# vovach777/llcomp

Hardware: AMD Instinct MI355X
Metric: encode+decode MPix/s on 4K RGB8, bit-exact (higher is better)
Workload: dtype int32

## Files before the change

llcomp_amd/csrc/model_kernels.hip:

```cpp
#include <algorithm>

#include "device_common.hpp"
#include "kernels.hpp"

namespace llcomp_mi {

namespace {

constexpr int kMW = 256;
constexpr int kMH = 32;

template <int C>
__device__ __forceinline__ void rct_forward(const uint8_t* p, int16_t (&o)[C]) {
    if constexpr (C >= 3) {
        const int g = p[1], cb = int(p[2]) - g, cr = int(p[0]) - g;
        o[0] = int16_t(cr);
        o[1] = int16_t(g + (cb + cr) / 4);
        o[2] = int16_t(cb);
        if constexpr (C == 4) o[3] = p[3];
    } else {
#pragma unroll
        for (int k = 0; k < C; ++k) o[k] = p[k];
    }
}
// ... 500 lines not shown
constexpr uint32_t kSegPieceDwords = 4096;
__global__ __launch_bounds__(256) void k_copy_segments(const uint8_t* __restrict__ src, uint8_t* __restrict__ dst,
                                                       const uint64_t* __restrict__ src_off, const uint64_t* __restrict__ dst_off,
                                                       const uint64_t* __restrict__ len) {
    const uint64_t n = len[blockIdx.y];
    const uint8_t* s = src + src_off[blockIdx.y];
    uint8_t* d = dst + dst_off[blockIdx.y];
    const uint64_t head = min(n, uint64_t((4 - (reinterpret_cast<uintptr_t>(d) & 3)) & 3));
    const uint64_t ndw = (n - head) >> 2, tail = (n - head) & 3;
    for (uint64_t j0 = uint64_t(blockIdx.x) * kSegPieceDwords; j0 < ndw; j0 += uint64_t(gridDim.x) * kSegPieceDwords) {
        const uint64_t j1 = min(ndw, j0 + kSegPieceDwords);
        for (uint64_t j = j0 + threadIdx.x; j < j1; j += 256) {
            uint32_t w;
            __builtin_memcpy(&w, s + head + 4 * j, 4);
            *reinterpret_cast<uint32_t*>(d + head + 4 * j) = w;
        }
    }
    if (blockIdx.x == 0) {
        if (threadIdx.x < head) d[threadIdx.x] = s[threadIdx.x];
        if (threadIdx.x < tail) d[head + 4 * ndw + threadIdx.x] = s[head + 4 * ndw + threadIdx.x];
    }
}

__global__ __launch_bounds__(256) void k_range_sums(const uint32_t* __restrict__ vals, const uint64_t* __restrict__ start,
                                                    const uint64_t* __restrict__ count, uint64_t* __restrict__ out, uint32_t cap) {
    __shared__ unsigned long long part[4];
    const uint64_t s = start[blockIdx.x], n = count[blockIdx.x];
    unsigned long long acc = 0;
    for (uint64_t j = threadIdx.x; j < n; j += 256) acc += min(vals[s + j], cap);
    for (int o = 32; o > 0; o >>= 1) acc += __shfl_down(acc, o);
    if ((threadIdx.x & 63) == 0) part[threadIdx.x >> 6] = acc;
    __syncthreads();
    if (threadIdx.x == 0) out[blockIdx.x] = part[0] + part[1] + part[2] + part[3];
}

struct SliceSpan {
    unsigned long long origin;
    uint32_t n_row;
    uint32_t n;
};
__device__ __forceinline__ void load_spans(const Geometry& g, uint32_t group, SliceSpan* spans) {
    if (threadIdx.x < 64) {
        const uint32_t id = (group << g.lane_shift) + threadIdx.x;
        SliceSpan sp{0, 1, 0};
        if (threadIdx.x < (1u << g.lane_shift) && id < g.n_slices) {
            const SliceRect r = slice_rect(g, id);
            sp.origin = slice_origin(g, r);
            sp.n_row = r.sw * g.nch;
            sp.n = sp.n_row * r.sh;
        }
        spans[threadIdx.x] = sp;
    }
    __syncthreads();
}
__device__ __forceinline__ size_t span_index(const SliceSpan& sp, uint32_t k, size_t row_stride) {
    const uint32_t y = k / sp.n_row;
    return size_t(sp.origin) + size_t(y) * row_stride + (k - y * sp.n_row);
}

template <typename T>
__global__ __launch_bounds__(256) void k_to_lane_order(const Geometry g, const uint32_t max_n,
                                                       const T* __restrict__ img, T* __restrict__ lanes) {
    __shared__ SliceSpan spans[64];
    __shared__ T tile[64][65];
    const uint32_t chunks = (max_n + 63) / 64;
    const uint32_t group = blockIdx.x / chunks, k0 = (blockIdx.x - group * chunks) * 64;
    load_spans(g, group, spans);
    const size_t rs = slice_row_stride(g);
    const uint32_t a = threadIdx.x & 63, b = threadIdx.x >> 6;
    {
        T v[16];
#pragma unroll
        for (int t = 0; t < 16; ++t) {
            const SliceSpan sp = spans[b + 4 * t];
            const uint32_t k = k0 + a;
            v[t] = k < sp.n ? img[span_index(sp, k, rs)] : T(0);
        }
#pragma unroll
        for (int t = 0; t < 16; ++t) tile[b + 4 * t][a] = v[t];
    }
    __syncthreads();
    const uint32_t gw = 1u << g.lane_shift;
    T* out = lanes + ((size_t(group) * max_n + k0) << g.lane_shift);
    const uint32_t n_el = min(64u, max_n - k0) << g.lane_shift;
    for (uint32_t el = threadIdx.x; el < n_el; el += 256) out[el] = tile[el & (gw - 1)][el >> g.lane_shift];
}

template <typename T>
__global__ __launch_bounds__(256) void k_from_lane_order(const Geometry g, const uint32_t max_n,
                                                         const T* __restrict__ lanes, T* __restrict__ img) {
    __shared__ SliceSpan spans[64];
    __shared__ T tile[64][65];
    const uint32_t chunks = (max_n + 63) / 64;
    const uint32_t group = blockIdx.x / chunks, k0 = (blockIdx.x - group * chunks) * 64;
    load_spans(g, group, spans);
    const size_t rs = slice_row_stride(g);
    const uint32_t a = threadIdx.x & 63, b = threadIdx.x >> 6;
    const uint32_t gw = 1u << g.lane_shift;
    const T* in = lanes + ((size_t(group) * max_n + k0) << g.lane_shift);
    const uint32_t n_el = min(64u, max_n - k0) << g.lane_shift;
    {
        T v[16];
#pragma unroll
        for (int t = 0; t < 16; ++t) {
            const uint32_t el = threadIdx.x + 256 * t;
            v[t] = el < n_el ? in[el] : T(0);
        }
#pragma unroll
        for (int t = 0; t < 16; ++t) {
            const uint32_t el = threadIdx.x + 256 * t;
            if (el < (64u << g.lane_shift)) tile[el & (gw - 1)][el >> g.lane_shift] = v[t];
        }
    }
    __syncthreads();
    for (uint32_t j = b; j < 64; j += 4) {
        const SliceSpan sp = spans[j];
        const uint32_t k = k0 + a;
        if (k < sp.n) img[span_index(sp, k, rs)] = tile[j][a];
    }
}

constexpr uint32_t kXcds = 8;
__device__ __forceinline__ bool xcd_group_chunk(uint32_t n_groups, uint32_t chunks, uint32_t& group, uint32_t& chunk) {
    const uint32_t xcd = blockIdx.x % kXcds, slot = blockIdx.x / kXcds;
    group = (slot / chunks) * kXcds + xcd;
    chunk = slot - (slot / chunks) * chunks;
    return group < n_groups;
}
__host__ inline uint64_t xcd_grid(uint32_t n_groups, uint32_t chunks) { return uint64_t((n_groups + kXcds - 1) / kXcds) * kXcds * chunks; }
__device__ __forceinline__ bool xcd_chunk_group(uint32_t n_groups, uint32_t chunks, uint32_t& group, uint32_t& chunk) {
    const uint32_t xcd = blockIdx.x % kXcds, slot = blockIdx.x / kXcds;
    const uint32_t per_class = (chunks + kXcds - 1) / kXcds;
    group = slot / per_class;
    chunk = xcd + kXcds * (slot - group * per_class);
    return group < n_groups && chunk < chunks;
}
__host__ inline uint64_t xcd_chunk_grid(uint32_t n_groups, uint32_t chunks) { return uint64_t(n_groups) * ((chunks + kXcds - 1) / kXcds) * kXcds; }

template <int C>
__device__ __forceinline__ void rct_pixel(const uint8_t* p, int (&v)[C]) {
    if constexpr (C >= 3) {
        const int g = p[1], cb = int(p[2]) - g, cr = int(p[0]) - g;
        v[0] = cr;
        v[1] = g + (cb + cr) / 4;
        v[2] = cb;
        if constexpr (C == 4) v[3] = p[3];
    } else {
#pragma unroll
        for (int k = 0; k < C; ++k) v[k] = p[k];
    }
}
struct RowTile {
    unsigned long long base;
    uint32_t sw;
};
template <int C>
__device__ __forceinline__ void load_row_tiles(const Geometry& g, uint32_t first_tile, uint32_t ntiles, RowTile* tiles) {
    if (threadIdx.x < ntiles) {
        const uint32_t tile = first_tile + threadIdx.x;
        const uint32_t per_frame = g.ntx * g.nty;
        const uint32_t frame = tile / per_frame, rem = tile - frame * per_frame;
        const uint32_t y = rem / g.ntx, tx = rem - y * g.ntx;
        const uint32_t x0 = tx * g.tile_w;
        tiles[threadIdx.x].base = ((size_t(frame) * g.h + y) * g.w + x0) * C;
        tiles[threadIdx.x].sw = g.w - x0 < g.tile_w ? g.w - x0 : g.tile_w;
    }
}

typedef short s16x2 __attribute__((ext_vector_type(2)));
typedef unsigned short u16x2 __attribute__((ext_vector_type(2)));
__device__ __forceinline__ u16x2 pk_min_u16(u16x2 a, u16x2 b) {
    u16x2 d;
    asm("v_pk_min_u16 %0, %1, %2" : "=v"(d) : "v"(a), "v"(b));
    return d;
}

template <int C>
__global__ __launch_bounds__(256) void k_model_rows_fwd(const Geometry g, const uint8_t* __restrict__ px,
                                                        uint16_t* __restrict__ lanes) {
    constexpr int K = 64, RUN = (K + 2) * C, TPG = 64 / C + 2;
    constexpr int RUNW = (RUN + 3) / 4 + 1;
    constexpr int PADL = (C - 1 + 1) & ~1, OCOLS = (PADL + 64 + C - 1 + 1) & ~1;
    __shared__ uint32_t raw[TPG][RUNW + 1];
    __shared__ __attribute__((aligned(4))) uint16_t otile[K][OCOLS];
    __shared__ RowTile tiles[TPG];
    const uint32_t chunks = (g.tile_w + K - 1) / K;
    uint32_t group, chunk;
    if (!xcd_group_chunk((g.n_slices + (1u << g.lane_shift) - 1) >> g.lane_shift, chunks, group, chunk)) return;
    const uint32_t k0 = chunk * K;
    const uint32_t gw = 1u << g.lane_shift;
    const uint32_t first_id = group << g.lane_shift;
    const uint32_t end_id = first_id + gw < g.n_slices ? first_id + gw : g.n_slices;
    const uint32_t first_tile = first_id / C, ntiles = (end_id - 1) / C - first_tile + 1;
    load_row_tiles<C>(g, first_tile, ntiles, tiles);
    __syncthreads();
    const size_t total_bytes = size_t(g.frames) * g.h * g.w * C;
    const uint32_t lane = threadIdx.x & 63, wave = threadIdx.x >> 6;
    constexpr int TPW = (TPG + 3) / 4, DPT = (RUNW + 63) / 64;
    uint32_t got[TPW][DPT];
#pragma unroll
    for (int t = 0; t < TPW; ++t) {
        const uint32_t tt = wave + 4 * t;
#pragma unroll
        for (int e = 0; e < DPT; ++e) got[t][e] = 0;
        if (tt < ntiles) {
            const long long start = (long long)tiles[tt].base + (long long)(int(k0) - 2) * C;
            const unsigned long long a0u = (unsigned long long)(start & ~3ll);
            const long long a0 = (long long)((unsigned long long)uint32_t(__builtin_amdgcn_readfirstlane(uint32_t(a0u))) |
                                             ((unsigned long long)uint32_t(__builtin_amdgcn_readfirstlane(uint32_t(a0u >> 32))) << 32));
            if (a0 >= 0 && size_t(a0) + 4 * size_t(RUNW) <= total_bytes) {
#pragma unroll
                for (int e = 0; e < DPT; ++e) {
                    const uint32_t d = lane + 64 * e;
                    if (d < uint32_t(RUNW)) __builtin_memcpy(&got[t][e], px + a0 + 4 * d, 4);
                }
            } else {
#pragma unroll
                for (int e = 0; e < DPT; ++e) {
                    const long long al = a0 + 4ll * (lane + 64 * e);
                    if (al >= 0 && size_t(al) + 4 <= total_bytes) __builtin_memcpy(&got[t][e], px + al, 4);
                    else if (al >= 0 && size_t(al) < total_bytes) got[t][e] = load_bytes_le(px + al, uint32_t(total_bytes - size_t(al)));
                }
            }
        }
    }
#pragma unroll
    for (int t = 0; t < TPW; ++t) {
        const uint32_t tt = wave + 4 * t;
#pragma unroll
        for (int e = 0; e < DPT; ++e) {
            const uint32_t d = lane + 64 * e;
            if (tt < ntiles && d < uint32_t(RUNW)) raw[tt][d] = got[t][e];
        }
    }
    __syncthreads();
    const uint32_t q = threadIdx.x & 7;
    const bool small = (g.flags & kGeoSmallModel) != 0;
    for (uint32_t tt = threadIdx.x >> 3; tt < ntiles; tt += 32) {
        const uint32_t sw = tiles[tt].sw;
        const uint32_t kb = k0 + 8 * q;
        if (kb >= sw) continue;
        const uint32_t skew = uint32_t(((long long)tiles[tt].base + (long long)(int(k0) - 2) * C) & 3);
        const uint8_t* p = reinterpret_cast<const uint8_t*>(&raw[tt][0]) + skew + 8 * q * C;
        s16x2 V[C][5];
#pragma unroll
        for (int j = 0; j < 5; ++j) {
            const uint8_t* a = p + 2 * j * C;
            if constexpr (C >= 3) {
                const s16x2 R = {short(a[0]), short(a[C])}, G = {short(a[1]), short(a[C + 1])}, B = {short(a[2]), short(a[C + 2])};
                const s16x2 cr = R - G, cb = B - G, sum = cb + cr;
                V[0][j] = cr;
                V[1][j] = G + ((sum + ((sum >> 15) & short(3))) >> 2);
                V[2][j] = cb;
                if constexpr (C == 4) V[3][j] = s16x2{short(a[3]), short(a[C + 3])};
            } else {
#pragma unroll
                for (int ch = 0; ch < C; ++ch) V[ch][j] = s16x2{short(a[ch]), short(a[C + ch])};
            }
        }
        uint32_t first_mask = ~0u;
        if (kb == 0) {
            first_mask = 0;
#pragma unroll
            for (int ch = 0; ch < C; ++ch) V[ch][0] = s16x2{128, 128};
        }
        if (small) first_mask = 0;
        const uint32_t colp = uint32_t(int((first_tile + tt) * C) - int(first_id) + PADL);
#pragma unroll
        for (int m = 0; m < 4; ++m) {
#pragma unroll
            for (int ch = 0; ch < C; ++ch) {
                const s16x2 cur = V[ch][m + 1], Lp = V[ch][m];
                const s16x2 lp = {V[ch][m].y, V[ch][m + 1].x};
                s16x2 dq = Lp - lp;
                uint32_t dqb = __builtin_bit_cast(uint32_t, dq) & ((m == 0 || small) ? first_mask : ~0u);
                dq = __builtin_bit_cast(s16x2, dqb);
                const s16x2 neg = dq >> 15;
                const u16x2 aq = __builtin_bit_cast(u16x2, (dq ^ neg) - neg);
                const u16x2 one = {1, 1};
                const u16x2 cidx = pk_min_u16(aq, one) + pk_min_u16(aq >> 2, one);
                const s16x2 res = ((cur - lp) ^ neg) - neg;
                const u16x2 sym = (__builtin_bit_cast(u16x2, res) & (unsigned short)0xFFF) + (cidx << 12);
                otile[8 * q + 2 * m][colp + ch] = sym.x;
                otile[8 * q + 2 * m + 1][colp + ch] = sym.y;
            }
        }
    }
    __syncthreads();
    if (g.lane_shift == 6) {
        for (uint32_t i = threadIdx.x; i < uint32_t(K) * 32; i += 256) {
            const uint32_t kk = i >> 5, d = i & 31, k = k0 + kk;
            if (k < g.tile_w)
                *reinterpret_cast<uint32_t*>(lanes + lane_order_index(g, first_id + 2 * d, k)) =
                    *reinterpret_cast<const uint32_t*>(&otile[kk][PADL + 2 * d]);
        }
    } else {
        for (uint32_t i = threadIdx.x; i < uint32_t(K) * gw; i += 256) {
            const uint32_t kk = i / gw, col = i - kk * gw, k = k0 + kk;
            if (k < g.tile_w && first_id + col < end_id) lanes[lane_order_index(g, first_id + col, k)] = otile[kk][PADL + col];
        }
    }
}

template <int C>
__global__ __launch_bounds__(256) void k_model_rows_inv(const Geometry g, const int16_t* __restrict__ lanes,
                                                        uint8_t* __restrict__ px) {
    constexpr int K = 64, TPG = 64 / C + 2;
    __shared__ __attribute__((aligned(4))) int16_t tile[K][64 + C + 1 + ((C + 1) & 1)];
    __shared__ RowTile tiles[TPG];
    const uint32_t chunks = (g.tile_w + K - 1) / K;
    uint32_t group, chunk;
    if (!xcd_chunk_group((g.n_slices + (1u << g.lane_shift) - 1) >> g.lane_shift, chunks, group, chunk)) return;
    const uint32_t k0 = chunk * K;
    const uint32_t gw = 1u << g.lane_shift;
    const uint32_t first_id = group << g.lane_shift;
    const uint32_t end_id = first_id + gw < g.n_slices ? first_id + gw : g.n_slices;
    const uint32_t first_tile = (first_id + C - 1) / C;
    const uint32_t end_tile = (end_id + C - 1) / C;
    if (first_tile >= end_tile) return;
    const uint32_t ntiles = end_tile - first_tile;
    load_row_tiles<C>(g, first_tile, ntiles, tiles);
    {
        uint32_t w[K * 32 / 256];
#pragma unroll
        for (int it = 0; it < K * 32 / 256; ++it) {
            const uint32_t i = threadIdx.x + 256 * it, kk = i >> 5, d = i & 31, k = k0 + kk;
            w[it] = 0;
            if (k < g.tile_w && g.lane_shift == 6)
                w[it] = *reinterpret_cast<const uint32_t*>(lanes + lane_order_index(g, first_id + 2 * d, k));
        }
        static_assert(K * (C - 1) <= 256, "one extra lane sample per thread");
        const uint32_t xk = threadIdx.x / (C > 1 ? C - 1 : 1), xe = threadIdx.x - xk * (C - 1);
        int16_t x = 0;
        if constexpr (C > 1) {
            const uint32_t id = first_id + gw + xe;
            if (xk < uint32_t(K) && id < g.n_slices && k0 + xk < g.tile_w) x = lanes[lane_order_index(g, id, k0 + xk)];
        }
#pragma unroll
        for (int it = 0; it < K * 32 / 256; ++it) {
            const uint32_t i = threadIdx.x + 256 * it, kk = i >> 5, d = i & 31;
            *reinterpret_cast<uint32_t*>(&tile[kk][2 * d]) = w[it];
        }
        if (g.lane_shift != 6) {
            __syncthreads();
            for (uint32_t i = threadIdx.x; i < uint32_t(K) * gw; i += 256) {
                const uint32_t kk = i / gw, col = i - kk * gw, k = k0 + kk;
                tile[kk][col] = (first_id + col < g.n_slices && k < g.tile_w) ? lanes[lane_order_index(g, first_id + col, k)] : int16_t(0);
            }
        }
        if constexpr (C > 1) {
            if (xk < uint32_t(K)) tile[xk][gw + xe] = x;
        }
    }
    __syncthreads();
    const uint32_t col0 = first_tile * C - first_id;
    const uint32_t q4 = threadIdx.x & 15;
    for (uint32_t tt = threadIdx.x >> 4; tt < ntiles; tt += 16) {
        const uint32_t sw = tiles[tt].sw, kb = k0 + 4 * q4;
        if (kb >= sw) continue;
        uint8_t bytes[4 * C];
#pragma unroll
        for (int i = 0; i < 4; ++i) {
            const int16_t* s = &tile[4 * q4 + i][col0 + tt * C];
            if constexpr (C >= 3) {
                int r = s[0], gg = s[1], bb = s[2];
                gg -= (r + bb) / 4;
                r += gg;
                bb += gg;
                bytes[i * C + 0] = uint8_t(min(max(r, 0), 255));
                bytes[i * C + 1] = uint8_t(min(max(gg, 0), 255));
                bytes[i * C + 2] = uint8_t(min(max(bb, 0), 255));
                if constexpr (C == 4) bytes[i * C + 3] = uint8_t(s[3]);
            } else {
#pragma unroll
                for (int c = 0; c < C; ++c) bytes[i * C + c] = uint8_t(s[c]);
            }
        }
        uint8_t* o = px + tiles[tt].base + size_t(kb) * C;
        const uint32_t npx = sw - kb < 4 ? sw - kb : 4;
        if (npx == 4) {
            uint32_t w[C];
#pragma unroll
            for (int c = 0; c < C; ++c)
                w[c] = uint32_t(bytes[4 * c]) | (uint32_t(bytes[4 * c + 1]) << 8) | (uint32_t(bytes[4 * c + 2]) << 16) |
                       (uint32_t(bytes[4 * c + 3]) << 24);
            __builtin_memcpy(o, w, 4 * C);
        } else {
            for (uint32_t i = 0; i < npx * C; ++i) o[i] = bytes[i];
        }
    }
}

struct RowTileCrop {
    long long base;
    uint32_t klo, khi;
};
template <int C>
__device__ __forceinline__ void load_row_tiles_crop(const Geometry& g, uint32_t first_tile, uint32_t ntiles, const Crop& cr,
                                                    RowTileCrop* tiles) {
    if (threadIdx.x < ntiles) {
        const uint32_t tile = first_tile + threadIdx.x;
        const uint32_t per_frame = g.ntx * g.nty;
        const uint32_t frame = tile / per_frame, rem = tile - frame * per_frame;
        const uint32_t y = rem / g.ntx, tx = rem - y * g.ntx;
        const uint32_t x0 = tx * g.tile_w;
        const uint32_t sw = g.w - x0 < g.tile_w ? g.w - x0 : g.tile_w;
        const uint32_t klo = cr.x0 > x0 ? cr.x0 - x0 : 0u;
        uint32_t khi = cr.x0 + cr.rw > x0 ? min(sw, cr.x0 + cr.rw - x0) : 0u;
        if (y < cr.y0 || y >= cr.y0 + cr.rh || khi <= klo) khi = 0;
        tiles[threadIdx.x].base = ((long long)(size_t(frame) * cr.rh + (y - cr.y0)) * cr.rw + (long long)x0 - (long long)cr.x0) * C;
        tiles[threadIdx.x].klo = klo;
        tiles[threadIdx.x].khi = khi;
    }
}
template <int C>
__global__ __launch_bounds__(256) void k_model_rows_inv_crop(const Geometry g, const int16_t* __restrict__ lanes,
                                                             uint8_t* __restrict__ px, const Crop cr) {
    constexpr int K = 64, TPG = 64 / C + 2;
    __shared__ __attribute__((aligned(4))) int16_t tile[K][64 + C + 1 + ((C + 1) & 1)];
    __shared__ RowTileCrop tiles[TPG];
    const uint32_t chunks = (g.tile_w + K - 1) / K;
    uint32_t group, chunk;
    if (!xcd_chunk_group((g.n_slices + (1u << g.lane_shift) - 1) >> g.lane_shift, chunks, group, chunk)) return;
    const uint32_t k0 = chunk * K;
    const uint32_t gw = 1u << g.lane_shift;
    const uint32_t first_id = group << g.lane_shift;
    const uint32_t end_id = first_id + gw < g.n_slices ? first_id + gw : g.n_slices;
    const uint32_t first_tile = (first_id + C - 1) / C;
    const uint32_t end_tile = (end_id + C - 1) / C;
    if (first_tile >= end_tile) return;
    const uint32_t ntiles = end_tile - first_tile;
    load_row_tiles_crop<C>(g, first_tile, ntiles, cr, tiles);
    {
        uint32_t w[K * 32 / 256];
#pragma unroll
        for (int it = 0; it < K * 32 / 256; ++it) {
            const uint32_t i = threadIdx.x + 256 * it, kk = i >> 5, d = i & 31, k = k0 + kk;
            w[it] = 0;
            if (k < g.tile_w && g.lane_shift == 6)
                w[it] = *reinterpret_cast<const uint32_t*>(lanes + lane_order_index(g, first_id + 2 * d, k));
        }
#pragma unroll
        for (int it = 0; it < K * 32 / 256; ++it) {
            const uint32_t i = threadIdx.x + 256 * it, kk = i >> 5, d = i & 31;
            *reinterpret_cast<uint32_t*>(&tile[kk][2 * d]) = w[it];
        }
    }
    if (g.lane_shift != 6) {
        __syncthreads();
        for (uint32_t i = threadIdx.x; i < uint32_t(K) * gw; i += 256) {
            const uint32_t kk = i / gw, col = i - kk * gw, k = k0 + kk;
            tile[kk][col] = (first_id + col < g.n_slices && k < g.tile_w) ? lanes[lane_order_index(g, first_id + col, k)] : int16_t(0);
        }
    }
    if constexpr (C > 1) {
        for (uint32_t i = threadIdx.x; i < uint32_t(K) * (C - 1); i += 256) {
            const uint32_t kk = i / (C - 1), e = i - kk * (C - 1), k = k0 + kk;
            const uint32_t id = first_id + gw + e;
            tile[kk][gw + e] = (id < g.n_slices && k < g.tile_w) ? lanes[lane_order_index(g, id, k)] : int16_t(0);
        }
    }
    __syncthreads();
    const uint32_t col0 = first_tile * C - first_id;
    const uint32_t q4 = threadIdx.x & 15;
    for (uint32_t tt = threadIdx.x >> 4; tt < ntiles; tt += 16) {
        const uint32_t sw = tiles[tt].khi, klo = tiles[tt].klo, kb = k0 + 4 * q4;
        if (kb >= sw || kb + 4 <= klo) continue;
        uint8_t bytes[4 * C];
#pragma unroll
        for (int i = 0; i < 4; ++i) {
            const int16_t* s = &tile[4 * q4 + i][col0 + tt * C];
            if constexpr (C >= 3) {
                int r = s[0], gg = s[1], bb = s[2];
                gg -= (r + bb) / 4;
                r += gg;
                bb += gg;
                bytes[i * C + 0] = uint8_t(min(max(r, 0), 255));
                bytes[i * C + 1] = uint8_t(min(max(gg, 0), 255));
                bytes[i * C + 2] = uint8_t(min(max(bb, 0), 255));
                if constexpr (C == 4) bytes[i * C + 3] = uint8_t(s[3]);
            } else {
#pragma unroll
                for (int c = 0; c < C; ++c) bytes[i * C + c] = uint8_t(s[c]);
            }
        }
        const uint32_t npx = sw - kb < 4 ? sw - kb : 4;
        if (npx < 4 || kb < klo) {
            for (uint32_t i = kb < klo ? klo - kb : 0u; i < npx; ++i)
                for (uint32_t c = 0; c < uint32_t(C); ++c) px[tiles[tt].base + (long long)(kb + i) * C + c] = bytes[i * C + c];
            continue;
        }
        uint32_t w[C];
#pragma unroll
        for (int c = 0; c < C; ++c)
            w[c] = uint32_t(bytes[4 * c]) | (uint32_t(bytes[4 * c + 1]) << 8) | (uint32_t(bytes[4 * c + 2]) << 16) |
                   (uint32_t(bytes[4 * c + 3]) << 24);
        __builtin_memcpy(px + tiles[tt].base + size_t(kb) * C, w, 4 * C);
    }
}



__global__ __launch_bounds__(256) void k_regions_index(const Geometry full, const Geometry sub, const RegionsFrame* __restrict__ tab,
                                                       const uint32_t* __restrict__ slice_len, const uint64_t* __restrict__ group_off,
                                                       uint32_t* __restrict__ sub_len, uint64_t* __restrict__ sub_off) {
    const uint32_t j = blockIdx.x * 256 + threadIdx.x;
    if (j >= sub.n_slices) return;
    const uint32_t id = regions_full_id(full, sub, tab, j);
    unsigned long long o = group_off[id >> full.lane_shift];
    for (uint32_t i = id & ~((1u << full.lane_shift) - 1); i < id; ++i) o += slice_len[i];
    sub_len[j] = slice_len[id];
    sub_off[j] = o;
}

template <int C>
__global__ __launch_bounds__(256) void k_model_inv_crops(const Geometry g, const int16_t* __restrict__ rec, uint8_t* __restrict__ px,
                                                         const RegionsFrame* __restrict__ tab, uint32_t rw, uint32_t rh, size_t npix) {
    const uint32_t c = C ? uint32_t(C) : g.c;
    const size_t per_frame = size_t(rw) * rh;
    for (size_t i = size_t(blockIdx.x) * blockDim.x + threadIdx.x; i < npix; i += size_t(gridDim.x) * blockDim.x) {
        const uint32_t f = uint32_t(i / per_frame);
        const uint32_t rem = uint32_t(i - f * per_frame), yy = rem / rw, xx = rem - yy * rw;
        const uint32_t y = tab[f].cy0 + yy, x = tab[f].cx0 + xx;
        uint8_t* o = px + (size_t(tab[f].out) * per_frame + rem) * c;
        uint32_t k = 0;
        if (c >= 3) {
            int r = rec[sample_index(g, f, y, x, 0)], gg = rec[sample_index(g, f, y, x, 1)], b = rec[sample_index(g, f, y, x, 2)];
            gg -= (r + b) / 4;
            r += gg;
            b += gg;
            o[0] = uint8_t(min(max(r, 0), 255));
            o[1] = uint8_t(min(max(gg, 0), 255));
            o[2] = uint8_t(min(max(b, 0), 255));
            k = 3;
        }
        for (; k < c; ++k) o[k] = uint8_t(rec[sample_index(g, f, y, x, k)]);
    }
}

template <int C>
__device__ __forceinline__ void load_row_tiles_crops(const Geometry& g, uint32_t first_tile, uint32_t ntiles, const RegionsFrame* tab,
                                                     uint32_t rw, uint32_t rh, RowTileCrop* tiles) {
    if (threadIdx.x < ntiles) {
        const uint32_t tile = first_tile + threadIdx.x;
        const uint32_t per_frame = g.ntx * g.nty;
        const uint32_t frame = tile / per_frame, rem = tile - frame * per_frame;
        const uint32_t y = rem / g.ntx, tx = rem - y * g.ntx;
        const uint32_t x0 = tx * g.tile_w;
        const uint32_t sw = g.w - x0 < g.tile_w ? g.w - x0 : g.tile_w;
        const uint32_t cx0 = tab[frame].cx0, cy0 = tab[frame].cy0;
        const uint32_t klo = cx0 > x0 ? cx0 - x0 : 0u;
        uint32_t khi = cx0 + rw > x0 ? min(sw, cx0 + rw - x0) : 0u;
        if (y < cy0 || y >= cy0 + rh || khi <= klo) khi = 0;
        tiles[threadIdx.x].base = ((long long)(size_t(tab[frame].out) * rh + (y - cy0)) * rw + (long long)x0 - (long long)cx0) * C;
        tiles[threadIdx.x].klo = klo;
        tiles[threadIdx.x].khi = khi;
    }
}
template <int C>
__global__ __launch_bounds__(256) void k_model_rows_inv_crops(const Geometry g, const int16_t* __restrict__ lanes,
                                                              uint8_t* __restrict__ px, const RegionsFrame* __restrict__ tab,
                                                              uint32_t rw, uint32_t rh) {
    constexpr int K = 64, TPG = 64 / C + 2;
    __shared__ __attribute__((aligned(4))) int16_t tile[K][64 + C + 1 + ((C + 1) & 1)];
    __shared__ RowTileCrop tiles[TPG];
    const uint32_t chunks = (g.tile_w + K - 1) / K;
    uint32_t group, chunk;
    if (!xcd_chunk_group((g.n_slices + (1u << g.lane_shift) - 1) >> g.lane_shift, chunks, group, chunk)) return;
    const uint32_t k0 = chunk * K;
    const uint32_t gw = 1u << g.lane_shift;
    const uint32_t first_id = group << g.lane_shift;
    const uint32_t end_id = first_id + gw < g.n_slices ? first_id + gw : g.n_slices;
    const uint32_t first_tile = (first_id + C - 1) / C;
    const uint32_t end_tile = (end_id + C - 1) / C;
    if (first_tile >= end_tile) return;
    const uint32_t ntiles = end_tile - first_tile;
    load_row_tiles_crops<C>(g, first_tile, ntiles, tab, rw, rh, tiles);
    {
        uint32_t w[K * 32 / 256];
#pragma unroll
        for (int it = 0; it < K * 32 / 256; ++it) {
            const uint32_t i = threadIdx.x + 256 * it, kk = i >> 5, d = i & 31, k = k0 + kk;
            w[it] = 0;
            if (k < g.tile_w && g.lane_shift == 6)
                w[it] = *reinterpret_cast<const uint32_t*>(lanes + lane_order_index(g, first_id + 2 * d, k));
        }
#pragma unroll
        for (int it = 0; it < K * 32 / 256; ++it) {
            const uint32_t i = threadIdx.x + 256 * it, kk = i >> 5, d = i & 31;
            *reinterpret_cast<uint32_t*>(&tile[kk][2 * d]) = w[it];
        }
    }
    if (g.lane_shift != 6) {
        __syncthreads();
        for (uint32_t i = threadIdx.x; i < uint32_t(K) * gw; i += 256) {
            const uint32_t kk = i / gw, col = i - kk * gw, k = k0 + kk;
            tile[kk][col] = (first_id + col < g.n_slices && k < g.tile_w) ? lanes[lane_order_index(g, first_id + col, k)] : int16_t(0);
        }
    }
    if constexpr (C > 1) {
        for (uint32_t i = threadIdx.x; i < uint32_t(K) * (C - 1); i += 256) {
            const uint32_t kk = i / (C - 1), e = i - kk * (C - 1), k = k0 + kk;
            const uint32_t id = first_id + gw + e;
            tile[kk][gw + e] = (id < g.n_slices && k < g.tile_w) ? lanes[lane_order_index(g, id, k)] : int16_t(0);
        }
    }
    __syncthreads();
    const uint32_t col0 = first_tile * C - first_id;
    const uint32_t q4 = threadIdx.x & 15;
    for (uint32_t tt = threadIdx.x >> 4; tt < ntiles; tt += 16) {
        const uint32_t sw = tiles[tt].khi, klo = tiles[tt].klo, kb = k0 + 4 * q4;
        if (kb >= sw || kb + 4 <= klo) continue;
        uint8_t bytes[4 * C];
#pragma unroll
        for (int i = 0; i < 4; ++i) {
            const int16_t* s = &tile[4 * q4 + i][col0 + tt * C];
            if constexpr (C >= 3) {
                int r = s[0], gg = s[1], bb = s[2];
                gg -= (r + bb) / 4;
                r += gg;
                bb += gg;
                bytes[i * C + 0] = uint8_t(min(max(r, 0), 255));
                bytes[i * C + 1] = uint8_t(min(max(gg, 0), 255));
                bytes[i * C + 2] = uint8_t(min(max(bb, 0), 255));
                if constexpr (C == 4) bytes[i * C + 3] = uint8_t(s[3]);
            } else {
#pragma unroll
                for (int c = 0; c < C; ++c) bytes[i * C + c] = uint8_t(s[c]);
            }
        }
        const uint32_t npx = sw - kb < 4 ? sw - kb : 4;
        if (npx < 4 || kb < klo) {
            for (uint32_t i = kb < klo ? klo - kb : 0u; i < npx; ++i)
                for (uint32_t c = 0; c < uint32_t(C); ++c) px[tiles[tt].base + (long long)(kb + i) * C + c] = bytes[i * C + c];
            continue;
        }
        uint32_t w[C];
#pragma unroll
        for (int c = 0; c < C; ++c)
            w[c] = uint32_t(bytes[4 * c]) | (uint32_t(bytes[4 * c + 1]) << 8) | (uint32_t(bytes[4 * c + 2]) << 16) |
                   (uint32_t(bytes[4 * c + 3]) << 24);
        __builtin_memcpy(px + tiles[tt].base + size_t(kb) * C, w, 4 * C);
    }
}


}

#define LLMI_DISPATCH_C(c, CALL) \
    switch (c) {                 \
        case 1: { constexpr int C = 1; CALL; } break; \
        case 2: { constexpr int C = 2; CALL; } break; \
        case 3: { constexpr int C = 3; CALL; } break; \
        case 4: { constexpr int C = 4; CALL; } break; \
        default: return hipErrorInvalidValue; \
    }

hipError_t launch_model_fwd(const Geometry& g, const uint8_t* d_px, uint32_t* d_sym, hipStream_t stream) {
    if (g.c > 4) {
        const size_t npix = size_t(g.frames) * g.h * g.w;
        k_model_fwd_any<<<dim3(uint32_t((npix + 255) / 256)), dim3(256), 0, stream>>>(g, d_px, d_sym, npix);
        return hipGetLastError();
    }
    const uint32_t nbx = (g.w + kMW - 1) / kMW;
    const uint32_t spt = (g.tile_h + kMH - 1) / kMH;
    const uint64_t blocks = uint64_t(nbx) * spt * g.nty * g.frames;
    if (blocks == 0 || blocks > 0x7FFFFFFFull) return hipErrorInvalidValue;
    LLMI_DISPATCH_C(g.c, (k_model_fwd<C><<<dim3(uint32_t(blocks)), dim3(kMW), 0, stream>>>(g, d_px, d_sym)));
    return hipGetLastError();
}

uint32_t lane_groups(const Geometry& g) { return (g.n_slices + (1u << g.lane_shift) - 1) >> g.lane_shift; }
uint32_t slice_capacity_samples(const Geometry& g) { return g.slice_samples; }

hipError_t launch_to_lane_order_u32(const Geometry& g, const uint32_t* d_img, uint32_t* d_lanes, hipStream_t stream) {
    const uint32_t max_n = slice_capacity_samples(g);
    const uint64_t blocks = uint64_t(lane_groups(g)) * ((max_n + 63) / 64);
    if (blocks == 0 || blocks > 0x7FFFFFFFull) return hipErrorInvalidValue;
    k_to_lane_order<uint32_t><<<dim3(uint32_t(blocks)), dim3(256), 0, stream>>>(g, max_n, d_img, d_lanes);
    return hipGetLastError();
}

hipError_t launch_from_lane_order_i16(const Geometry& g, const int16_t* d_lanes, int16_t* d_img, hipStream_t stream) {
    const uint32_t max_n = slice_capacity_samples(g);
    const uint64_t blocks = uint64_t(lane_groups(g)) * ((max_n + 63) / 64);
    if (blocks == 0 || blocks > 0x7FFFFFFFull) return hipErrorInvalidValue;
    k_from_lane_order<int16_t><<<dim3(uint32_t(blocks)), dim3(256), 0, stream>>>(g, max_n, d_lanes, d_img);
    return hipGetLastError();
}

bool model_is_fused(const Geometry& g) { return g.planar && rows_mode(g) && g.c <= 4; }
bool rows_encoder_reads_pixels(const Geometry& g) {
    return model_is_fused(g) && (uint64_t(63 / g.c + 2) * g.tile_w * g.c + 4 < (1ull << 31));
}

hipError_t launch_model_rows_fwd(const Geometry& g, const uint8_t* d_px, uint16_t* d_lanes, hipStream_t stream) {
    const uint64_t blocks = xcd_grid(lane_groups(g), (g.tile_w + 63) / 64);
    if (blocks == 0 || blocks > 0x7FFFFFFFull) return hipErrorInvalidValue;
    LLMI_DISPATCH_C(g.c, (k_model_rows_fwd<C><<<dim3(uint32_t(blocks)), dim3(256), 0, stream>>>(g, d_px, d_lanes)));
    return hipGetLastError();
}

hipError_t launch_model_rows_inv(const Geometry& g, const int16_t* d_lanes, uint8_t* d_px, hipStream_t stream) {
    const uint64_t blocks = xcd_chunk_grid(lane_groups(g), (g.tile_w + 63) / 64);
    if (blocks == 0 || blocks > 0x7FFFFFFFull) return hipErrorInvalidValue;
    LLMI_DISPATCH_C(g.c, (k_model_rows_inv<C><<<dim3(uint32_t(blocks)), dim3(256), 0, stream>>>(g, d_lanes, d_px)));
    return hipGetLastError();
}

hipError_t launch_model_inv(const Geometry& g, const int16_t* d_rec, uint8_t* d_px, hipStream_t stream) {
    const size_t npix = size_t(g.frames) * g.h * g.w;
    if (g.c > 4) {
        k_model_inv_any<<<dim3(uint32_t((npix + 255) / 256)), dim3(256), 0, stream>>>(g, d_rec, d_px, npix);
        return hipGetLastError();
    }
    const uint32_t blocks = uint32_t(std::min<size_t>((npix + 255) / 256, 256 * 16));
    LLMI_DISPATCH_C(g.c, (k_model_inv<C><<<dim3(blocks), dim3(256), 0, stream>>>(g, d_rec, d_px, npix)));
    return hipGetLastError();
}

hipError_t launch_group_sums(const Geometry& g, const uint32_t* d_slice_len, uint64_t* d_group_off, hipStream_t stream) {
    k_group_sums<<<dim3((g.n_slices + kSumThreads - 1) / kSumThreads), dim3(kSumThreads), 0, stream>>>(d_slice_len, g.n_slices, g.lane_shift, d_group_off);
    return hipGetLastError();
}

hipError_t launch_frame_bytes(const Geometry& g, const uint32_t* d_slice_len, uint64_t* d_frame_bytes, hipStream_t stream) {
    k_frame_bytes<<<dim3(g.frames), dim3(256), 0, stream>>>(d_slice_len, g.slices_per_frame, d_frame_bytes);
    return hipGetLastError();
}

hipError_t launch_scan_groups(const Geometry& g, uint64_t* d_group_off, uint64_t* d_total, hipStream_t stream) {
    k_scan_groups<<<dim3(1), dim3(kScanThreads), 0, stream>>>(d_group_off, lane_groups(g), d_total);
    return hipGetLastError();
}

hipError_t launch_copy_segments(const uint8_t* d_src, uint8_t* d_dst, const uint64_t* d_src_off, const uint64_t* d_dst_off,
                                const uint64_t* d_len, uint32_t n_seg, uint64_t max_len, hipStream_t stream) {
    if (n_seg == 0) return hipSuccess;
    if (n_seg > 65535) return hipErrorInvalidValue;
    const uint64_t pieces = (max_len / 4 + kSegPieceDwords - 1) / kSegPieceDwords;
    const uint32_t gx = uint32_t(std::min<uint64_t>(std::max<uint64_t>(pieces, 1), 1024));
    k_copy_segments<<<dim3(gx, n_seg), dim3(256), 0, stream>>>(d_src, d_dst, d_src_off, d_dst_off, d_len);
    return hipGetLastError();
}

hipError_t launch_range_sums(const uint32_t* d_vals, const uint64_t* d_start, const uint64_t* d_count, uint64_t* d_out, uint32_t n,
                             uint32_t cap, hipStream_t stream) {
    if (!n) return hipSuccess;
    k_range_sums<<<dim3(n), dim3(256), 0, stream>>>(d_vals, d_start, d_count, d_out, cap);
    return hipGetLastError();
}

hipError_t launch_pack_payload(const Geometry& g, const uint8_t* d_units, const uint32_t* d_slice_len,
                               const uint64_t* d_offsets, uint8_t* d_payload, uint64_t payload_cap,
                               uint32_t* d_status, hipStream_t stream) {
    k_pack_payload<<<dim3(lane_groups(g)), dim3(256), 0, stream>>>(g, reinterpret_cast<const uint4*>(d_units), d_slice_len,
                                                                   d_offsets, d_payload, payload_cap, d_status);
    return hipGetLastError();
}

hipError_t launch_region_index(const Geometry& full, const Geometry& sub, const RegionBox& box, const uint32_t* d_slice_len,
                               const uint64_t* d_group_off, uint32_t* d_sub_len, uint64_t* d_sub_off, hipStream_t stream) {
    if (sub.n_slices == 0) return hipErrorInvalidValue;
    k_region_index<<<dim3((sub.n_slices + 255) / 256), dim3(256), 0, stream>>>(full, sub, box, d_slice_len, d_group_off, d_sub_len, d_sub_off);
    return hipGetLastError();
}

hipError_t launch_stage_region_streams(const Geometry& sub, const uint8_t* d_payload, uint64_t payload_bytes, const uint32_t* d_sub_len,
                                       const uint64_t* d_sub_off, uint8_t* d_units, uint32_t* d_status, hipStream_t stream) {
    k_stage_region_streams<<<dim3(lane_groups(sub)), dim3(256), 0, stream>>>(sub, d_payload, payload_bytes, d_sub_len, d_sub_off,
                                                                             reinterpret_cast<uint4*>(d_units), d_status);
    return hipGetLastError();
}

hipError_t launch_model_inv_crop(const Geometry& sub, const int16_t* d_rec, uint8_t* d_px, const Crop& cr, hipStream_t stream) {
    const size_t npix = size_t(sub.frames) * cr.rh * cr.rw;
    if (npix == 0 || uint64_t(cr.x0) + cr.rw > sub.w || uint64_t(cr.y0) + cr.rh > sub.h) return hipErrorInvalidValue;
    const uint32_t blocks = uint32_t(std::min<size_t>((npix + 255) / 256, 256 * 16));
    switch (sub.c) {
        case 1: k_model_inv_crop<1><<<dim3(blocks), dim3(256), 0, stream>>>(sub, d_rec, d_px, cr, npix); break;
        case 2: k_model_inv_crop<2><<<dim3(blocks), dim3(256), 0, stream>>>(sub, d_rec, d_px, cr, npix); break;
        case 3: k_model_inv_crop<3><<<dim3(blocks), dim3(256), 0, stream>>>(sub, d_rec, d_px, cr, npix); break;
        case 4: k_model_inv_crop<4><<<dim3(blocks), dim3(256), 0, stream>>>(sub, d_rec, d_px, cr, npix); break;
        default: k_model_inv_crop<0><<<dim3(blocks), dim3(256), 0, stream>>>(sub, d_rec, d_px, cr, npix); break;
    }
    return hipGetLastError();
}

hipError_t launch_model_rows_inv_crop(const Geometry& sub, const int16_t* d_lanes, uint8_t* d_px, const Crop& cr, hipStream_t stream) {
    if (!cr.rw || !cr.rh || uint64_t(cr.x0) + cr.rw > sub.w || uint64_t(cr.y0) + cr.rh > sub.h) return hipErrorInvalidValue;
    const uint64_t blocks = xcd_chunk_grid(lane_groups(sub), (sub.tile_w + 63) / 64);
    if (blocks == 0 || blocks > 0x7FFFFFFFull) return hipErrorInvalidValue;
    LLMI_DISPATCH_C(sub.c, (k_model_rows_inv_crop<C><<<dim3(uint32_t(blocks)), dim3(256), 0, stream>>>(sub, d_lanes, d_px, cr)));
    return hipGetLastError();
}

hipError_t launch_regions_index(const Geometry& full, const Geometry& sub, const RegionsFrame* d_tab, const uint32_t* d_slice_len,
                                const uint64_t* d_group_off, uint32_t* d_sub_len, uint64_t* d_sub_off, hipStream_t stream) {
    if (sub.n_slices == 0) return hipErrorInvalidValue;
    k_regions_index<<<dim3((sub.n_slices + 255) / 256), dim3(256), 0, stream>>>(full, sub, d_tab, d_slice_len, d_group_off, d_sub_len, d_sub_off);
    return hipGetLastError();
}

hipError_t launch_model_inv_crops(const Geometry& sub, const int16_t* d_rec, uint8_t* d_px, const RegionsFrame* d_tab, uint32_t rw,
                                  uint32_t rh, hipStream_t stream) {
    const size_t npix = size_t(sub.frames) * rh * rw;
    if (npix == 0 || rw > sub.w || rh > sub.h) return hipErrorInvalidValue;
    const uint32_t blocks = uint32_t(std::min<size_t>((npix + 255) / 256, 256 * 16));
    switch (sub.c) {
        case 1: k_model_inv_crops<1><<<dim3(blocks), dim3(256), 0, stream>>>(sub, d_rec, d_px, d_tab, rw, rh, npix); break;
        case 2: k_model_inv_crops<2><<<dim3(blocks), dim3(256), 0, stream>>>(sub, d_rec, d_px, d_tab, rw, rh, npix); break;
        case 3: k_model_inv_crops<3><<<dim3(blocks), dim3(256), 0, stream>>>(sub, d_rec, d_px, d_tab, rw, rh, npix); break;
        case 4: k_model_inv_crops<4><<<dim3(blocks), dim3(256), 0, stream>>>(sub, d_rec, d_px, d_tab, rw, rh, npix); break;
        default: k_model_inv_crops<0><<<dim3(blocks), dim3(256), 0, stream>>>(sub, d_rec, d_px, d_tab, rw, rh, npix); break;
    }
    return hipGetLastError();
}

hipError_t launch_model_rows_inv_crops(const Geometry& sub, const int16_t* d_lanes, uint8_t* d_px, const RegionsFrame* d_tab, uint32_t rw,
                                       uint32_t rh, hipStream_t stream) {
    if (!rw || !rh || rw > sub.w || rh > sub.h) return hipErrorInvalidValue;
    const uint64_t blocks = xcd_chunk_grid(lane_groups(sub), (sub.tile_w + 63) / 64);
    if (blocks == 0 || blocks > 0x7FFFFFFFull) return hipErrorInvalidValue;
    LLMI_DISPATCH_C(sub.c, (k_model_rows_inv_crops<C><<<dim3(uint32_t(blocks)), dim3(256), 0, stream>>>(sub, d_lanes, d_px, d_tab, rw, rh)));
    return hipGetLastError();
}

hipError_t launch_stage_streams(const Geometry& g, const uint8_t* d_payload, uint64_t payload_bytes,
                                const uint32_t* d_slice_len, const uint64_t* d_offsets, uint8_t* d_units,
                                uint32_t* d_status, hipStream_t stream) {
    k_stage_streams<<<dim3(lane_groups(g)), dim3(256), 0, stream>>>(g, d_payload, payload_bytes, d_slice_len, d_offsets,
                                                                    reinterpret_cast<uint4*>(d_units), d_status);
    return hipGetLastError();
}

}
```

Before: 31010.

## Run rows inverse kernel as single-wavefront blocks with wave-level LDS ordering

Shrinks the inverse rows kernel from 256-thread blocks to one 64-lane wavefront per block and moves its shared memory to a dynamically sized struct. Block-wide __syncthreads is replaced by a wavefront fence plus wave barrier. The lane-load path now issues unpredicated loads with clamped indices into registers, waits on the memory counter, then writes LDS. The aim is to remove block-barrier cost and predicate overhead and to let more small blocks stay resident, at the cost of more work per thread and a dependence on load_row_tiles being correct with 64 threads.

```diff
diff --git a/llcomp_amd/csrc/model_kernels.hip b/llcomp_amd/csrc/model_kernels.hip
--- a/llcomp_amd/csrc/model_kernels.hip
+++ b/llcomp_amd/csrc/model_kernels.hip
@@ -826,12 +826,24 @@
     }
 }
 
+__device__ __forceinline__ void wave_lds_order() {
+    __builtin_amdgcn_fence(__ATOMIC_ACQ_REL, "wavefront");
+    __builtin_amdgcn_wave_barrier();
+}
+
 template <int C>
-__global__ __launch_bounds__(256) void k_model_rows_inv(const Geometry g, const int16_t* __restrict__ lanes,
-                                                        uint8_t* __restrict__ px) {
+struct RowsInvLds {
+    int16_t tile[64][64 + C + 1 + ((C + 1) & 1)];
+    RowTile tiles[64 / C + 2];
+};
+extern __shared__ __attribute__((aligned(16))) uint8_t rows_inv_lds[];
+template <int C>
+__global__ __launch_bounds__(64) void k_model_rows_inv(const Geometry g, const int16_t* __restrict__ lanes,
+                                                       uint8_t* __restrict__ px) {
     constexpr int K = 64, TPG = 64 / C + 2;
-    __shared__ __attribute__((aligned(4))) int16_t tile[K][64 + C + 1 + ((C + 1) & 1)];
-    __shared__ RowTile tiles[TPG];
+    RowsInvLds<C>& lds = *reinterpret_cast<RowsInvLds<C>*>(rows_inv_lds);
+    int16_t (&tile)[K][64 + C + 1 + ((C + 1) & 1)] = lds.tile;
+    RowTile (&tiles)[TPG] = lds.tiles;
     const uint32_t chunks = (g.tile_w + K - 1) / K;
     uint32_t group, chunk;
     if (!xcd_chunk_group((g.n_slices + (1u << g.lane_shift) - 1) >> g.lane_shift, chunks, group, chunk)) return;
@@ -844,42 +856,45 @@
     if (first_tile >= end_tile) return;
     const uint32_t ntiles = end_tile - first_tile;
     load_row_tiles<C>(g, first_tile, ntiles, tiles);
-    {
-        uint32_t w[K * 32 / 256];
-#pragma unroll
-        for (int it = 0; it < K * 32 / 256; ++it) {
-            const uint32_t i = threadIdx.x + 256 * it, kk = i >> 5, d = i & 31, k = k0 + kk;
-            w[it] = 0;
-            if (k < g.tile_w && g.lane_shift == 6)
-                w[it] = *reinterpret_cast<const uint32_t*>(lanes + lane_order_index(g, first_id + 2 * d, k));
-        }
-        static_assert(K * (C - 1) <= 256, "one extra lane sample per thread");
-        const uint32_t xk = threadIdx.x / (C > 1 ? C - 1 : 1), xe = threadIdx.x - xk * (C - 1);
-        int16_t x = 0;
+    if (g.lane_shift == 6) {
+        const uint32_t last = min(uint32_t(K), g.tile_w - k0) - 1;
+        const uint32_t d = threadIdx.x & 31, hi = threadIdx.x >> 5;
+        const uint32_t* const rows = reinterpret_cast<const uint32_t*>(lanes + lane_order_index(g, first_id, k0));
+        uint32_t w[K / 2];
+#pragma unroll
+        for (int it = 0; it < K / 2; ++it) w[it] = rows[min(2 * it + hi, last) * 32 + d];
+        constexpr int XPL = C - 1;
+        int16_t x[XPL > 0 ? XPL : 1];
         if constexpr (C > 1) {
-            const uint32_t id = first_id + gw + xe;
-            if (xk < uint32_t(K) && id < g.n_slices && k0 + xk < g.tile_w) x = lanes[lane_order_index(g, id, k0 + xk)];
-        }
-#pragma unroll
-        for (int it = 0; it < K * 32 / 256; ++it) {
-            const uint32_t i = threadIdx.x + 256 * it, kk = i >> 5, d = i & 31;
-            *reinterpret_cast<uint32_t*>(&tile[kk][2 * d]) = w[it];
-        }
-        if (g.lane_shift != 6) {
-            __syncthreads();
-            for (uint32_t i = threadIdx.x; i < uint32_t(K) * gw; i += 256) {
-                const uint32_t kk = i / gw, col = i - kk * gw, k = k0 + kk;
-                tile[kk][col] = (first_id + col < g.n_slices && k < g.tile_w) ? lanes[lane_order_index(g, first_id + col, k)] : int16_t(0);
-            }
-        }
+            const bool next = first_id + 64 < g.n_slices;
+            const int16_t* const xrows = lanes + lane_order_index(g, next ? first_id + 64 : first_id, k0);
+            const uint32_t xlast = next ? min(uint32_t(C - 1), g.n_slices - first_id - 64) - 1 : 0;
+#pragma unroll
+            for (int j = 0; j < XPL; ++j) {
+                const uint32_t e = threadIdx.x + 64 * j, xk = e / (C - 1), xe = e - xk * (C - 1);
+                x[j] = xrows[min(xk, last) * 64 + min(xe, xlast)];
+            }
+        }
+        __builtin_amdgcn_s_waitcnt(0x0F70);
+#pragma unroll
+        for (int it = 0; it < K / 2; ++it) *reinterpret_cast<uint32_t*>(&tile[2 * it + hi][2 * d]) = w[it];
         if constexpr (C > 1) {
-            if (xk < uint32_t(K)) tile[xk][gw + xe] = x;
-        }
-    }
-    __syncthreads();
+#pragma unroll
+            for (int j = 0; j < XPL; ++j) {
+                const uint32_t e = threadIdx.x + 64 * j, xk = e / (C - 1), xe = e - xk * (C - 1);
+                tile[xk][64 + xe] = x[j];
+            }
+        }
+    } else {
+        for (uint32_t i = threadIdx.x; i < uint32_t(K) * (gw + C - 1); i += 64) {
+            const uint32_t kk = i / (gw + C - 1), col = i - kk * (gw + C - 1), k = k0 + kk;
+            tile[kk][col] = (first_id + col < g.n_slices && k < g.tile_w) ? lanes[lane_order_index(g, first_id + col, k)] : int16_t(0);
+        }
+    }
+    wave_lds_order();
     const uint32_t col0 = first_tile * C - first_id;
     const uint32_t q4 = threadIdx.x & 15;
-    for (uint32_t tt = threadIdx.x >> 4; tt < ntiles; tt += 16) {
+    for (uint32_t tt = threadIdx.x >> 4; tt < ntiles; tt += 4) {
         const uint32_t sw = tiles[tt].sw, kb = k0 + 4 * q4;
         if (kb >= sw) continue;
         uint8_t bytes[4 * C];
@@ -1228,7 +1243,7 @@
 hipError_t launch_model_rows_inv(const Geometry& g, const int16_t* d_lanes, uint8_t* d_px, hipStream_t stream) {
     const uint64_t blocks = xcd_chunk_grid(lane_groups(g), (g.tile_w + 63) / 64);
     if (blocks == 0 || blocks > 0x7FFFFFFFull) return hipErrorInvalidValue;
-    LLMI_DISPATCH_C(g.c, (k_model_rows_inv<C><<<dim3(uint32_t(blocks)), dim3(256), 0, stream>>>(g, d_lanes, d_px)));
+    LLMI_DISPATCH_C(g.c, (k_model_rows_inv<C><<<dim3(uint32_t(blocks)), dim3(64), sizeof(RowsInvLds<C>), stream>>>(g, d_lanes, d_px)));
     return hipGetLastError();
 }
 
```

Result: slower. 30670 (-1.1%).
